# linusmossberg/monte-carlo-ray-tracer

Measured on AMD Instinct MI355X. Metric: Mray/s (whole node), 1920x1080 @ 256 spp path trace, higher is better.
Workload: dtype f64; 1 GPU; hexagon_room.json cam0 1920x1080 @ 256 spp (BASELINE configs[1]); width=1920, height=1080, spp=256, integrator=path_tracer, seed=305419896, frame_finite=True

## Files before the change

monte-carlo-ray-tracer_amd/csrc/mcrt_hip.hip:

```cpp
#include <hip/hip_runtime.h>

#include <algorithm>
#include <chrono>
#include <cstdio>
#include <cstring>
#include <map>
#include <memory>
#include <mutex>
#include <string>
#include <vector>

#include "../../include/mcrt.h"
#include "mcrt_integrator.hpp"
#include "mcrt_lanesm.hpp"
#include "mcrt_qbvh.hpp"
#include "mcrt_wavefront.hpp"
#include "mcrt_waveknn.hpp"
#include "mcrt_groupknn.hpp"
#include "mcrt_widerec.hpp"
#include "mcrt_layout.hpp"
#include "mcrt_internal.hpp"
#include "mcrt_aov.hpp"
#include "mcrt_plan.hpp"
#include "mcrt_select.hpp"
// ... 583 lines not shown
    DeviceOrder& o = g_device_order[(unsigned)ctx->device & 63u];
    std::lock_guard<std::mutex> guard(o.m);
    if (gpu_wait && o.owner && o.owner != ctx) {
        HIP_TRY(ctx, hipSetDevice(ctx->device));
        HIP_TRY(ctx, hipStreamWaitEvent(stream, o.last, 0));
    }
    const int rc = launchRenderImpl(ctx, cam, global_seed, integrator, d_out, stream, film_out, opt);
    if (rc == MCRT_OK && ctx->pending) {
        o.last = ctx->ev1;
        o.owner = ctx;
        if (cam != &ctx->last_cam) ctx->last_cam = *cam;
        ctx->last_seed = global_seed;
        ctx->last_integrator = integrator;
        ctx->last_out = d_out;
        ctx->last_film = film_out;
        ctx->last_stream = stream;
    }
    return rc;
}

int launchRenderImpl(mcrt_ctx* ctx, const mcrt_camera_desc* cam, uint32_t global_seed, int integrator, double* d_out, hipStream_t stream,
                     double* film_out, const RenderOptions& opt) {
    if (!ctx->has_scene) return fail(ctx, MCRT_ERR_NO_SCENE, "mcrt_render before mcrt_upload_scene");
    if (int rc = validateCamera(ctx, cam)) return rc;
    const bool photon = integrator == MCRT_INTEGRATOR_PHOTON_MAPPER;
    if (integrator != MCRT_INTEGRATOR_PATH_TRACER && !photon) return fail(ctx, MCRT_ERR_INVALID, "unknown integrator");
    if (photon && !ctx->has_photons) return fail(ctx, MCRT_ERR_NO_PHOTONS, "photon mapping render before mcrt_upload_photons");
    if (ctx->pending) return fail(ctx, MCRT_ERR_INVALID, "a render is already in flight: call mcrt_render_finish");
    HIP_TRY(ctx, hipSetDevice(ctx->device));
    ctx->lean_used = false;

    const uint32_t owned_rows = mcrt_shard_rows(cam, nullptr);
    FrameFacts frame;
    frame.photon = photon;
    frame.paths = (uint64_t)owned_rows * cam->width * cam->sqrtspp * cam->sqrtspp;
    frame.filtered = filmSplats(cam->film_filter, cam->film_radius);
    frame.film_out = film_out != nullptr;
    frame.k_nearest = ctx->k_nearest;
    frame.max_lds = (uint32_t)ctx->max_lds;
    frame.force_wf = ctx->force_wf;
    frame.force_pm_lane = ctx->force_pm_lane;
    const KernelChoice choice = selectKernel(ctx->facts, frame, opt);
    if (choice.err != MCRT_OK) return fail(ctx, choice.err, choice.message);
    if (choice.form == MCRT_KERNEL_WAVEFRONT || choice.form == MCRT_KERNEL_WAVEFRONT_PM)
        return launchWavefront(ctx, cam, global_seed, d_out, stream, opt, choice, film_out);

    const void* kernel = instanceAddress(choice.instance, choice.lean);
    if (!kernel) return fail(ctx, MCRT_ERR_INVALID, "internal error: no such lean kernel instance");
    const bool pm_wave = choice.form == MCRT_KERNEL_PM_WAVE;
    const bool flat_karg = choice.instance == kInstFlatK512 || choice.instance == kInstFlatK768;
    DeviceScene launch_scene = ctx->scene;
    const uint32_t lds_bytes = planMegaLds(launch_scene, choice, (uint32_t)ctx->max_lds);
    if (lds_bytes > ctx->max_lds) return fail(ctx, MCRT_ERR_INVALID, "LDS plan exceeds the device limit");
    LaunchGeom g;
    if (int rc = occupancyGrid(ctx, kernel, choice.block, lds_bytes, g)) return rc;
    if (int rc = ensureScratch(ctx, g.total_lanes, photon && !pm_wave)) return rc;
    if (int rc = ensureSpill(ctx, megaSpillEntries(ctx->scene, choice, g.total_lanes) * sizeof(StackEntry))) return rc;
    if (int rc = beginFrame(ctx, stream, owned_rows == 0 ? (uint32_t)MCRT_KERNEL_NONE : choice.form)) return rc;
    if (owned_rows == 0) return endFrame(ctx, stream);
    ctx->lean_used = choice.lean;

    PassPlan pp;
    if (int rc = planSampleStore(ctx, opt.sample_store_gb, cam->width, owned_rows, cam->sqrtspp * cam->sqrtspp, pp)) return rc;
    RenderParams prm;
    fillRenderParams(prm, *cam, global_seed, owned_rows, ctx->work_counter.as<unsigned long long>(), ctx->stats.as<unsigned long long>(),
                     ctx->spill.as<StackEntry>(), ctx->samples.as<double>(), g.total_lanes);
    if (photon) {
        setRenderMaps(prm, ctx->maps[0], ctx->maps[1], ctx->k_nearest, ctx->direct_visualization);
        prm.knn_res_d2 = ctx->knn_res_d2.as<double>();
        prm.knn_res_idx = ctx->knn_res_idx.as<uint32_t>();
        prm.knn_visit_d2 = ctx->knn_visit_d2.as<double>();
        prm.knn_visit_oct = ctx->knn_visit_oct.as<uint32_t>();
        prm.knn_max_visit = ctx->knn_visit_alloc;
    }
    PmExtra pmx;
    if (pm_wave) {
        HIP_TRY(ctx, ctx->pm_stage.reserve(pmStageBytes(g.total_lanes)));
        HIP_TRY(ctx, ctx->knn_spill.reserve(pmKnnSpillBytes(g.total_lanes)));
        if (pmIorsInMemory(choice)) HIP_TRY(ctx, ctx->pm_iors.reserve(pmIorsBytes(g.total_lanes)));
        fillPmExtra(pmx, waveMapView(ctx, 0), waveMapView(ctx, 1), choice, ctx->pm_stage.as<double>(), ctx->knn_spill.as<uint32_t>(), ctx->pm_iors.as<double>());
    }
    FlatPreArg pre;
    if (flat_karg) {
        memset(&pre, 0, sizeof(pre));
        memcpy(pre.v, ctx->flat_pre_host.data(), ctx->flat_pre_host.size() * sizeof(float));
    }
    for (uint32_t row = 0; row < owned_rows; row += pp.pass_rows) {
        setRenderPass(prm, row, pp.pass_rows, photon, opt.chunks);
        const uint32_t grid = (uint32_t)std::min<uint64_t>(g.grid, (prm.work_items + g.block - 1) / g.block);
        HIP_TRY(ctx, hipMemsetAsync(ctx->work_counter.p, 0, sizeof(unsigned long long), stream));
        if (pm_wave)
            hipLaunchKernelGGL(kernelAs<PmKernelT>(kernel), dim3(grid), dim3(g.block), g.lds_bytes, stream, launch_scene, prm, pmx);
        else if (flat_karg)
            hipLaunchKernelGGL(kernelAs<FlatKernelT>(kernel), dim3(grid), dim3(g.block), g.lds_bytes, stream, launch_scene, prm, pre);
        else
            hipLaunchKernelGGL(kernelAs<RenderKernelT>(kernel), dim3(grid), dim3(g.block), g.lds_bytes, stream, launch_scene, prm);
        ctx->launches++;
        if (int rc = launchPassEpilogue(ctx, stream, prm.samples, prm.pass_pixels, prm.spp, d_out, prm.row_base, cam->width)) return rc;
    }
    return endFrame(ctx, stream);
}


int planSampleStore(mcrt_ctx* ctx, double store_gb, uint32_t width, uint32_t owned_rows, uint32_t spp, PassPlan& pp) {
    double gb = store_gb;
    size_t free_b = 0, total_b = 0;
    if (hipMemGetInfo(&free_b, &total_b) == hipSuccess) gb = std::min(gb, 0.4 * (double)(free_b + ctx->samples.bytes) / 1e9);
    else (void)hipGetLastError();
    for (;;) {
        pp = planPasses(width, owned_rows, spp, gb);
        if (ctx->samples.bytes >= pp.store_bytes) return MCRT_OK;
        if (ctx->samples.alloc(pp.store_bytes) == hipSuccess) return MCRT_OK;
        (void)hipGetLastError();
        if (pp.pass_rows <= 8) return fail(ctx, MCRT_ERR_HIP, "out of device memory for the per-sample store of one 8-row pass");
        gb = std::min(gb, (double)pp.store_bytes / 1e9) * 0.5;
    }
}

int uploadMap(mcrt_ctx* ctx, int which, const mcrt_photon_map_desc* m) {
    PhotonMapView& v = ctx->maps[which];
    memset(&v, 0, sizeof(v));
    ctx->map_children_ptr[which] = nullptr;
    if (!m || m->num_octants == 0 || m->num_photons == 0) return MCRT_OK;
    if (m->num_photons > 0xFFFFFFFEull) return fail(ctx, MCRT_ERR_UNSUPPORTED, "photon map larger than 2^32-2 photons per GPU");
    if (!m->octant_bounds || !m->octant_start_data || !m->octant_contained_data || !m->octant_next_sibling || !m->octant_leaf || !m->photons)
        return fail(ctx, MCRT_ERR_INVALID, "photon map descriptor has null arrays");
    const size_t n = m->num_octants;
    std::vector<uint32_t> start(n), contained(n);
    for (size_t i = 0; i < n; i++) {
        if (m->octant_start_data[i] + m->octant_contained_data[i] > m->num_photons)
            return fail(ctx, MCRT_ERR_INVALID, "photon map octant range exceeds the photon array");
        start[i] = (uint32_t)m->octant_start_data[i];
        contained[i] = (uint32_t)m->octant_contained_data[i];
    }
    if (int rc = uploadArray(ctx, ctx->map_bounds[which], m->octant_bounds, n * 6)) return rc;
    if (int rc = uploadArray(ctx, ctx->map_start[which], start.data(), n)) return rc;
    if (int rc = uploadArray(ctx, ctx->map_contained[which], contained.data(), n)) return rc;
    if (int rc = uploadArray(ctx, ctx->map_next[which], m->octant_next_sibling, n)) return rc;
    if (int rc = uploadArray(ctx, ctx->map_leaf[which], m->octant_leaf, n)) return rc;
    if (int rc = uploadArray(ctx, ctx->map_photons[which], m->photons, (size_t)m->num_photons * 8)) return rc;
    {
        std::vector<WideRec> wide;
        uint32_t root_a = 0, root_m = 0;
        const int wrc = buildWideRecords(m, contained.data(), std::max<uint32_t>(ctx->k_nearest, 1u), wide, root_a, root_m);
        if (wrc == 1) return fail(ctx, MCRT_ERR_INVALID, "photon octant with more than 8 children");
        if (wrc == 2) return fail(ctx, MCRT_ERR_UNSUPPORTED, "photon map too large for 32-bit record indices");
        if (int rc = uploadArray(ctx, ctx->map_children[which], wide.data(), wide.size())) return rc;
        ctx->map_children_ptr[which] = ctx->map_children[which].as<WideRec>();
        ctx->map_root_a[which] = root_a;
        ctx->map_root_m[which] = root_m;
    }
    v.num_octants = m->num_octants;
    v.num_photons = m->num_photons;
    v.octant_bounds = ctx->map_bounds[which].as<double>();
    v.octant_start = ctx->map_start[which].as<uint32_t>();
    v.octant_contained = ctx->map_contained[which].as<uint32_t>();
    v.octant_next = ctx->map_next[which].as<uint32_t>();
    v.octant_leaf = ctx->map_leaf[which].as<uint8_t>();
    v.photons = ctx->map_photons[which].as<float>();
    return buildMapPositions(ctx, which, m->num_photons);
}

#include "mcrt_photon_device.hpp"

}

// ... 894 lines not shown
```

monte-carlo-ray-tracer_amd/csrc/mcrt_launch.hpp:

```cpp
#ifndef MCRT_LAUNCH_FRAME_SECTION
#define MCRT_LAUNCH_FRAME_SECTION

#include <algorithm>
#include <cstring>
#include <vector>

#include "../../include/mcrt.h"
#include "mcrt_plan.hpp"
#include "mcrt_wavefront.hpp"

namespace mcrt {

inline std::vector<double> filmCacheTable(const mcrt_camera_desc& cam) {
    std::vector<double> table(cam.film_cache_size);
    for (uint32_t i = 0; i < cam.film_cache_size; i++)
        table[i] = filmFilterFunction(filmViewType(cam.film_filter), (2.0 * (int)i) / (double)(cam.film_cache_size - 1));
    return table;
}
inline FilmView makeFilmView(const mcrt_camera_desc& cam, const double* cache, double* blob) {
    FilmView f;
    f.type = filmViewType(cam.film_filter);
    f.width = cam.width;
    f.height = cam.height;
    f.radius = cam.film_radius > 0.0 ? cam.film_radius : filmDefaultRadius(cam.film_filter);
    f.two_inv_radius = 2.0 / f.radius;
    f.cache_size = cam.film_cache_size;
    f.cache = f.cache_size ? cache : nullptr;
    f.inv_dx = f.cache_size ? (double)(f.cache_size - 1) / f.radius : 0.0;
    f.blob = blob;
    return f;
}

inline void fillWfFrame(WfFrame& fr, const mcrt_camera_desc& cam, uint32_t global_seed, const ChunkPlan& cp, double* samples, const FilmView* film,
                        double* iors_deep, uint32_t iors_depth) {
    memset(&fr, 0, sizeof(fr));
    fr.cam = cam;
    fr.global_seed = global_seed;
    fr.spp = cam.sqrtspp * cam.sqrtspp;
    fr.tiles_x = (cam.width + 7) / 8;
    fr.chunk_shift = cp.shift;
    fr.chunk = cp.chunk;
    fr.samples = samples;
    fr.film.type = MCRT_FILM_BOX;
    if (film) fr.film = *film;
    fr.iors_deep = iors_deep;
    fr.iors_deep_rows = iors_depth - (uint32_t)kMaxIors;
}
inline void setWfPass(WfFrame& fr, uint32_t row_base, uint32_t row_end) {
    fr.row_base = row_base;
    fr.row_end = row_end;
    fr.pass_pixels = (unsigned long long)(row_end - row_base) * fr.cam.width;
    fr.work_items = ((unsigned long long)fr.tiles_x * ((row_end - row_base + 7) / 8) * 64ull) << fr.chunk_shift;
}

inline std::vector<double> lightFlux(const mcrt_scene_desc& s) {
    std::vector<double> flux((size_t)s.num_lights * 3);
    for (uint32_t i = 0; i < s.num_lights; i++) {
        const uint32_t ls = s.light_surface[i];
        for (int c = 0; c < 3; c++) flux[(size_t)i * 3 + c] = s.materials[s.surf_material[ls]].emittance[c] * s.surf_area[ls];
    }
    return flux;
}
inline void planEmission(const std::vector<double>& flux, double emissions, double caustic_factor, std::vector<unsigned long long>& first,
                         std::vector<double>& photon_flux) {
    const size_t nl = flux.size() / 3, photon_emissions = (size_t)((double)(size_t)emissions * caustic_factor);
    double total_add_flux = 0.0;
    for (size_t i = 0; i < nl; i++) total_add_flux += 0.0 + flux[i * 3] + flux[i * 3 + 1] + flux[i * 3 + 2];
    first.assign(nl + 1, 0ull);
    photon_flux.resize(nl * 3);
    for (size_t i = 0; i < nl; i++) {
        const double* f = &flux[i * 3];
        const double share = (0.0 + f[0] + f[1] + f[2]) / total_add_flux;
        const size_t n = (size_t)((double)photon_emissions * share);
        first[i + 1] = first[i] + n;
        for (int c = 0; c < 3; c++) photon_flux[i * 3 + c] = f[c] / (double)n;
    }
}

}
#endif

#if defined(MCRT_LAUNCH_KERNEL_ARGS) && !defined(MCRT_LAUNCH_KERNEL_SECTION)
#define MCRT_LAUNCH_KERNEL_SECTION

inline void planStaging(DeviceScene& d, uint32_t max_lds, uint32_t flat_max, const HostLayout& L) {
    d.stage_all = 1;
    d.stage_nodes = 0;
    const uint32_t fixed = planLds(DeviceScene{}, kBlock).total;
    if (planLds(d, kBlock).total - fixed > 48u * 1024u || planLds(d, kBlock).total > max_lds || L.num_quadric_surfaces) {
        d.stage_all = 0;
        d.stage_nodes = std::min<uint32_t>(d.num_nodes, 512u);
    }
    d.flat = (d.stage_all && d.num_surfaces <= flat_max && !L.flat_prim.empty() && L.num_quadric_surfaces == 0) ? 1u : 0u;
}

constexpr uint32_t kPmStageNodes = 128;

inline SceneFacts sceneFacts(const DeviceScene& d, const HostLayout& L, const mcrt_scene_desc& s) {
    SceneFacts facts;
    facts.material_flags = 0u;
    for (uint32_t i = 0; i < s.num_materials; i++) facts.material_flags |= s.materials[i].flags;
    facts.q_single = L.q_single;
    facts.flat = d.flat != 0;
    facts.cull = d.flat_pre != nullptr;
    facts.cull_floats = L.flat_pre.size() == (size_t)d.pre_tri_pairs * kTriPairFloats + (size_t)d.pre_sph_pairs * kSphPairFloats ? (uint32_t)L.flat_pre.size() : 0u;
    facts.stage_all = d.stage_all != 0;
    facts.num_nodes = d.num_nodes;
    facts.q_nodes = d.q_nodes;
    DeviceScene pm = d;
    if (!pm.stage_all) pm.stage_nodes = std::min<uint32_t>(pm.stage_nodes, kPmStageNodes);
    for (uint32_t i = 0; i < 8; i++) {
        facts.pm_lds[0][i] = alignUp(planLds(pm, kBlock, true, 2 * (i + 1), kPmLdsIors).total, 16);
        facts.pm_lds[1][i] = alignUp(planLds(pm, 1024u, true, 2 * (i + 1), kPmLdsIors).total, 16);
    }
    facts.pm_lds_full = alignUp(planLds(pm, kBlock, true, kLdsStackDepth, kMaxIors).total, 16);
    return facts;
}

inline bool pmWide(const KernelChoice& c) { return c.instance >= kInstPMWide && c.instance <= kInstPMWide_CountAll; }
inline bool pmIorsInMemory(const KernelChoice& c) { return c.form == MCRT_KERNEL_PM_WAVE && (c.block == 1024u || pmWide(c)); }

inline uint32_t planMegaLds(DeviceScene& launch_scene, const KernelChoice& c, uint32_t max_lds) {
    if (c.form == MCRT_KERNEL_PM_WAVE) {
        if (!launch_scene.stage_all) launch_scene.stage_nodes = std::min<uint32_t>(launch_scene.stage_nodes, kPmStageNodes);
        const uint32_t knn_bytes = waveKnnBytes(pmWide(c) ? kWaveRowsLarge : kWaveRows) + (launch_scene.stage_all ? 0u : kWaveStateBytes);
        return alignUp(planLds(launch_scene, c.block, true, c.stack_depth, pmIorsInMemory(c) ? kPmLdsIors : (uint32_t)kMaxIors).total, 16) + (c.block / 64) * knn_bytes;
    }
    if (c.form == MCRT_KERNEL_LANE_SM) {
        const uint32_t fixed = planSmLds(DeviceScene{}, c.block, c.stack_depth).total;
        if (!launch_scene.stage_all && fixed < max_lds) launch_scene.stage_nodes = std::min<uint32_t>(launch_scene.stage_nodes, (max_lds - fixed) / 64u);
        return planSmLds(launch_scene, c.block, c.stack_depth).total;
    }
    return planLds(launch_scene, c.block, c.form != MCRT_KERNEL_FLAT).total;
}
inline size_t megaSpillEntries(const DeviceScene& d, const KernelChoice& c, uint32_t total_lanes) {
    const uint32_t in_lds = c.form == MCRT_KERNEL_PM_WAVE ? std::min<uint32_t>(c.stack_depth, kLdsStackDepth) : (uint32_t)kLdsStackDepth;
    return (size_t)total_lanes * (d.stack_depth - in_lds);
}

constexpr int kSmShadeLanes = 40, kSmRegenLanes = 16, kSmMinTrav = 20, kSmLeafLanes = 32, kSmMinInner = 8;

inline void fillRenderParams(RenderParams& prm, const mcrt_camera_desc& cam, uint32_t global_seed, uint32_t owned_rows, unsigned long long* work_counter,
                             unsigned long long* stats, StackEntry* spill, double* samples, uint32_t total_lanes) {
    memset(&prm, 0, sizeof(prm));
    prm.cam = cam;
    prm.global_seed = global_seed;
    prm.spp = cam.sqrtspp * cam.sqrtspp;
    prm.owned_rows = owned_rows;
    prm.tiles_x = (cam.width + 7) / 8;
    prm.tiles_y = (owned_rows + 7) / 8;
    prm.work_items = (uint64_t)prm.tiles_x * prm.tiles_y * 64ull;
    prm.work_counter = work_counter;
    prm.stats = stats;
    prm.spill = spill;
    prm.samples = samples;
    prm.total_lanes = total_lanes;
    prm.sm_shade_lanes = kSmShadeLanes;
    prm.sm_regen_lanes = kSmRegenLanes;
    prm.sm_min_trav = kSmMinTrav;
    prm.sm_leaf_lanes = kSmLeafLanes;
    prm.sm_min_inner = kSmMinInner;
    prm.sm_lds_depth = kLdsStackDepth;
}
inline void setRenderMaps(RenderParams& prm, const PhotonMapView& global_map, const PhotonMapView& caustic_map, uint32_t k_nearest, int direct_visualization) {
    prm.global_map = global_map;
    prm.caustic_map = caustic_map;
    prm.k_nearest = k_nearest;
    prm.direct_visualization = direct_visualization ? 1u : 0u;
}
inline void setRenderPass(RenderParams& prm, uint32_t row, uint64_t pass_rows, bool photon, long long chunks = -1) {
    prm.row_base = row;
    prm.row_end = (uint32_t)std::min<uint64_t>(prm.owned_rows, row + pass_rows);
    prm.pass_pixels = (uint64_t)(prm.row_end - prm.row_base) * prm.cam.width;
    const ChunkPlan cp = photon ? planChunks(prm.spp, unitsWanted(prm.total_lanes, 128, prm.pass_pixels, chunks))
                                : planChunksMega(prm.spp, prm.total_lanes, prm.pass_pixels, chunks);
    prm.chunk_shift = cp.shift;
    prm.chunk = cp.chunk;
    const uint64_t tiles = (uint64_t)prm.tiles_x * ((prm.row_end - prm.row_base + 7) / 8);
    prm.work_items = (tiles * 64ull) << cp.shift;
}

inline size_t pmStageBytes(uint32_t total_lanes) { return (size_t)kStageDoubles * total_lanes * sizeof(double); }
inline size_t pmKnnSpillBytes(uint32_t total_lanes) { return (size_t)(total_lanes / 64) * kWaveSpill * 3 * sizeof(uint32_t); }
inline size_t pmIorsBytes(uint32_t total_lanes) { return (size_t)kMaxIors * total_lanes * sizeof(double); }
inline void fillPmExtra(PmExtra& pmx, const PhotonMapViewW& global_map, const PhotonMapViewW& caustic_map, const KernelChoice& c, double* stage,
                        uint32_t* knn_spill, double* iors_global) {
    pmx.global_map = global_map;
    pmx.caustic_map = caustic_map;
// ... 152 lines not shown
```

monte-carlo-ray-tracer_amd/csrc/mcrt_layout.hpp:

```cpp
#pragma once

#include <algorithm>
#include <cmath>
#include <cstdlib>
#include <cstring>
#include <string>
#include <vector>

#include "../../include/mcrt.h"
#include "mcrt_scene.hpp"
#include "mcrt_qbvh.hpp"
#include "mcrt_bvh_shared.hpp"

namespace mcrt {

constexpr size_t kFlatCopyMax = 4096;

struct HostLayout {
    std::vector<double> node_bounds;
    std::vector<NodeMeta> node_meta;
    std::vector<double> prim;
    std::vector<double> normal;
    std::vector<double> shade_rec;
    bool any_vn = false;
// ... 145 lines not shown
    std::vector<uint32_t> order;
    order.reserve(n);
    std::vector<uint32_t> first_child_new(n, 0), child_count(n, 0);
    order.push_back(0);
    for (size_t head = 0; head < order.size(); head++) {
        const uint32_t old = order[head];
        if (s->node_num_surfaces[old] != 0) continue;
        uint32_t c = old + 1, cnt = 0;
        first_child_new[head] = (uint32_t)order.size();
        while (c != 0 && c < n) {
            order.push_back(c);
            cnt++;
            if (order.size() > n) {
                err = "BVH node links are cyclic";
                return MCRT_ERR_INVALID;
            }
            c = s->node_next_sibling[c];
        }
        child_count[head] = cnt;
    }
    if (order.size() != n) {
        err = "BVH has unreachable nodes";
        return MCRT_ERR_INVALID;
    }
    for (uint32_t i = 0; i < n; i++) {
        const uint32_t old = order[i];
        memcpy(&bounds[(size_t)i * 6], s->node_bounds + (size_t)old * 6, 48);
        if (s->node_num_surfaces[old] != 0) {
            if ((uint64_t)s->node_start_surface[old] + s->node_num_surfaces[old] > s->num_surfaces) {
                err = "BVH leaf range exceeds the surface array";
                return MCRT_ERR_INVALID;
            }
            meta[i] = NodeMeta{s->node_start_surface[old], s->node_num_surfaces[old]};
        } else {
            meta[i] = NodeMeta{first_child_new[i], kInnerFlag | child_count[i]};
        }
    }
    return MCRT_OK;
}

inline void buildFlatCull(HostLayout& L, uint32_t ns) {
    L.flat_pre.clear();
    L.pre_tri_pairs = L.pre_sph_pairs = 0;
    const uint32_t nt = L.flat_tris, nsph = ns - nt;
    if (ns == 0) return;
    double lo[3] = {INFINITY, INFINITY, INFINITY}, hi[3] = {-INFINITY, -INFINITY, -INFINITY};
    auto grow = [&](const double* p, double r) {
        for (int a = 0; a < 3; a++) {
            lo[a] = std::min(lo[a], p[a] - r);
            hi[a] = std::max(hi[a], p[a] + r);
        }
    };
    for (uint32_t i = 0; i < ns; i++) {
        const double* r = &L.flat_prim[(size_t)i * kPrimStride];
        if (i < nt) {
            const double v1[3] = {r[0] + r[3], r[1] + r[4], r[2] + r[5]}, v2[3] = {r[0] + r[6], r[1] + r[7], r[2] + r[8]};
            grow(r, 0.0);
            grow(v1, 0.0);
            grow(v2, 0.0);
        } else {
            grow(r, fabs(r[3]));
        }
    }
    double H = 0.0;
    for (int a = 0; a < 3; a++) {
        if (!(fabs(lo[a]) <= 1e7) || !(fabs(hi[a]) <= 1e7)) return;
        L.pre_centre[a] = 0.5 * (lo[a] + hi[a]);
        H = std::max(H, 0.5 * (hi[a] - lo[a]));
    }
    if (!(H > 0.0)) return;
    L.pre_bound = 4.0 * H;
    const double u = ldexp(1.0, -24), bound = L.pre_bound;
    auto up = [](double x) {
        float f = (float)x;
        if ((double)f < x) f = nextafterf(f, INFINITY);
        return f;
    };
    auto down = [](double x) {
        float f = (float)x;
        if ((double)f > x) f = nextafterf(f, -INFINITY);
        return f;
    };
    auto len = [](const double* v) { return sqrt(v[0] * v[0] + v[1] * v[1] + v[2] * v[2]); };
    L.pre_tri_pairs = (nt + 1) / 2;
    L.pre_sph_pairs = (nsph + 1) / 2;
    L.flat_pre.assign((size_t)L.pre_tri_pairs * kTriPairFloats + (size_t)L.pre_sph_pairs * kSphPairFloats, 0.0f);
    for (uint32_t i = 0; i < 2 * L.pre_tri_pairs; i++) {
        float* q = &L.flat_pre[(size_t)(i / 2) * kTriPairFloats + (i & 1)];
        if (i >= nt) {
            q[2 * 9] = -INFINITY;
            continue;
        }
        const double* r = &L.flat_prim[(size_t)i * kPrimStride];
        double a[3];
        for (int c = 0; c < 3; c++) a[c] = r[c] - L.pre_centre[c];
        for (int c = 0; c < 3; c++) q[2 * c] = (float)a[c];
        for (int c = 0; c < 6; c++) q[2 * (3 + c)] = (float)r[3 + c];
        const double e1 = len(r + 3), e2 = len(r + 6), tmax = sqrt(3.0) * bound + len(a);
        const double k = 4.0 * u;
        double eu = k * 31.0 * e1 * e2 * e2 * tmax, ev = k * 31.0 * e1 * e1 * e2 * tmax, et = k * 31.0 * e1 * e1 * e2 * e2 * tmax;
        double ew = k * 40.0 * e1 * e2 * ((e1 + e2) * tmax + e1 * e2);
        const bool degenerate = !(e1 > 1e-12) || !(e2 > 1e-12) || !(eu > 1e-30) || !(ev > 1e-30) || !(et > 1e-30) || !(ew > 1e-30);
        if (degenerate) eu = ev = et = ew = INFINITY;
        q[2 * 9] = up(eu);
        q[2 * 10] = up(ev);
        q[2 * 11] = up(et);
        q[2 * 12] = up(ew);
    }
    float* sph = L.flat_pre.data() + (size_t)L.pre_tri_pairs * kTriPairFloats;
    for (uint32_t i = 0; i < 2 * L.pre_sph_pairs; i++) {
        float* q = &sph[(size_t)(i / 2) * kSphPairFloats + (i & 1)];
        if (i >= nsph) {
            q[2 * 3] = -INFINITY;
            q[2 * 4] = 0.0f;
            continue;
        }
        const double* r = &L.flat_prim[(size_t)(nt + i) * kPrimStride];
        double c[3], cinf = 0.0;
        for (int a = 0; a < 3; a++) {
            c[a] = r[a] - L.pre_centre[a];
            cinf = std::max(cinf, fabs(c[a]));
            q[2 * a] = (float)c[a];
        }
        const double rad = fabs(r[3]), M = bound + cinf;
        const double beta = 4.0 * (12.0 * u + 7.0 * u * M / rad), gamma = 4.0 * (2.0 * u * rad * rad + 7.0 * u * rad * M);
        if (!(rad > 0.0) || !(beta < 0.25) || !(gamma > 1e-30)) {
            q[2 * 3] = INFINITY;
            q[2 * 4] = 0.0f;
        } else {
            q[2 * 3] = up(rad * rad + gamma);
            q[2 * 4] = down(1.0 - beta);
        }
    }
}


inline void synthRangeTree(const mcrt_scene_desc* s, std::vector<double>& bounds, std::vector<uint32_t>& start, std::vector<uint32_t>& count,
                           std::vector<uint32_t>& next) {
    const uint32_t ns = s->num_surfaces;
    std::vector<double> sb((size_t)ns * 6);
    for (uint32_t i = 0; i < ns; i++) surfaceBounds(s->surf_kind[i], s->surf_v + (size_t)i * 9, s->quadrics, &sb[(size_t)i * 6]);
    struct Rec {
        static uint32_t build(uint32_t a, uint32_t b, const std::vector<double>& sb, std::vector<double>& bounds, std::vector<uint32_t>& start,
                              std::vector<uint32_t>& count, std::vector<uint32_t>& next) {
            const uint32_t me = (uint32_t)start.size();
            double bb[6] = {1.7976931348623157e308, 1.7976931348623157e308, 1.7976931348623157e308,
                            -1.7976931348623157e308, -1.7976931348623157e308, -1.7976931348623157e308};
            for (uint32_t i = a; i < b; i++)
                for (int c = 0; c < 3; c++) {
                    bb[c] = sb[(size_t)i * 6 + c] < bb[c] ? sb[(size_t)i * 6 + c] : bb[c];
                    bb[3 + c] = sb[(size_t)i * 6 + 3 + c] > bb[3 + c] ? sb[(size_t)i * 6 + 3 + c] : bb[3 + c];
                }
            bounds.insert(bounds.end(), bb, bb + 6);
            start.push_back(a);
            next.push_back(0u);
            if (b - a <= 4u) {
                count.push_back(b - a);
                return me;
            }
            count.push_back(0u);
            const uint32_t part = (b - a + 3u) / 4u;
            uint32_t prev = 0;
            for (uint32_t x = a; x < b; x += part) {
                const uint32_t child = build(x, x + part < b ? x + part : b, sb, bounds, start, count, next);
                if (prev) next[prev] = child;
                prev = child;
            }
            return me;
        }
    };
    bounds.clear();
    start.clear();
    count.clear();
    next.clear();
    if (ns) Rec::build(0u, ns, sb, bounds, start, count, next);
}

inline int buildLayout(const mcrt_scene_desc* s, HostLayout& L, std::string& err) {
    const size_t ns = s->num_surfaces;
    L.prim.assign(ns * kPrimStride, 0.0);
    L.normal.assign(ns * 3, 0.0);
    L.any_vn = false;
    L.num_quadric_surfaces = 0;
    L.surf_v_patched.clear();
    for (size_t i = 0; i < ns; i++) {
        if (s->surf_material[i] >= s->num_materials) {
            err = "surface material index out of range";
            return MCRT_ERR_INVALID;
        }
        double* r = &L.prim[i * kPrimStride];
// ... 125 lines not shown
```

monte-carlo-ray-tracer_amd/csrc/mcrt_scene.hpp:

```cpp
#pragma once

#include "mcrt_math.hpp"

namespace mcrt {

constexpr uint32_t kInnerFlag = 0x80000000u;
constexpr int kPrimStride = 10;
constexpr int kLdsStackDepth = 16;
constexpr int kMaxStackDepth = 128;

struct NodeMeta {
    uint32_t a, b;
};

struct Node64 {
    double b[6];
    uint32_t a, m;
    uint32_t pad0, pad1;
};
constexpr uint32_t kSmInner = 0x100u;

struct Ray {
    d3 start, direction, inv_direction;
    double medium_ior, refraction_scale;
// ... 195 lines not shown
    const double tag = rec[9];
    if constexpr (kQuadrics) {
        if (tag == 3.0) return quadricIntersect(quadricPtr(rec[0]), ray, out);
    }
    if (tag == 1.0) {
        d3 so = ray.start - ld3(rec);
        double b = 2.0 * dot(ray.direction, so);
        double c = dot(so, so) - sq(rec[3]);
        double d = b * b - 4.0 * 1.0 * c;
        if (d < 0.0) return false;
        double sd = sqrt(d);
        double t = -0.5 * (b + (b < 0.0 ? -sd : sd));
        double t_min = t / 1.0;
        double t_max = c / t;
        if (t_min > t_max) {
            double tmp = t_min;
            t_min = t_max;
            t_max = tmp;
        }
        if (!(t_max >= 0.0)) return false;
        out.t = t_min < 0.0 ? t_max : t_min;
        out.u = 0.0;
        out.v = 0.0;
        out.interpolate = false;
        return true;
    }
    d3 v0 = ld3(rec), E1 = ld3(rec + 3), E2 = ld3(rec + 6);
    d3 P_ = cross(ray.direction, E2);
    double determinant = dot(P_, E1);
    if (determinant < kEpsilon && determinant > -kEpsilon) return false;
    double inv_determinant = 1.0 / determinant;
    d3 T = ray.start - v0;
    double u = dot(P_, T) * inv_determinant;
    if (u > 1.0 || u < 0.0) return false;
    d3 Q = cross(T, E1);
    double v = dot(Q, ray.direction) * inv_determinant;
    if (v > 1.0 || v < 0.0 || u + v > 1.0) return false;
    double t = dot(Q, E2) * inv_determinant;
    if (t <= 0.0) return false;
    out.t = t;
    out.interpolate = tag >= 2.0;
    out.u = out.interpolate ? u : 0.0;
    out.v = out.interpolate ? v : 0.0;
    return true;
}

MCRT_HD bool closer(double t, uint32_t surface, const Hit& best) {
    return t < best.t || (t == best.t && surface < best.surface);
}

template <class P>
MCRT_HD bool triangleTestFlat(P rec, d3 start, d3 direction, double& t, double& u, double& v) {
    d3 v0 = ld3(rec), E1 = ld3(rec + 3), E2 = ld3(rec + 6);
    d3 P_ = cross(direction, E2);
    double determinant = dot(P_, E1);
    double inv_determinant = 1.0 / determinant;
    d3 T = start - v0;
    u = dot(P_, T) * inv_determinant;
    d3 Q = cross(T, E1);
    v = dot(Q, direction) * inv_determinant;
    t = dot(Q, E2) * inv_determinant;
    const bool parallel = determinant < kEpsilon && determinant > -kEpsilon;
    const bool u_out = u > 1.0 || u < 0.0;
    const bool v_out = v > 1.0 || v < 0.0 || u + v > 1.0;
    return !parallel & !u_out & !v_out & !(t <= 0.0);
}
template <class P>
MCRT_HD bool sphereTestFlat(P rec, d3 start, d3 direction, double& t_hit) {
    d3 so = start - ld3(rec);
    double b = 2.0 * dot(direction, so);
    double c = dot(so, so) - sq(rec[3]);
    double d = b * b - 4.0 * 1.0 * c;
    double sd = sqrt(d);
    double t = -0.5 * (b + (b < 0.0 ? -sd : sd));
    double t_min = t / 1.0;
    double t_max = c / t;
    const bool swap = t_min > t_max;
    double lo = swap ? t_max : t_min, hi = swap ? t_min : t_max;
    t_hit = lo < 0.0 ? hi : lo;
    return !(d < 0.0) & (hi >= 0.0);
}

typedef float f2 __attribute__((vector_size(8)));
constexpr int kTriPairFloats = 32, kSphPairFloats = 16;
constexpr float kCullB2 = 1.0f + 8.0f * 5.9604645e-8f * 1.0001f;

template <class P>
MCRT_HD f2 ldf2(P p) {
    return f2{p[0], p[1]};
}

struct CullRay {
    f2 sx, sy, sz, dx, dy, dz;
    bool in_domain;
};
MCRT_HD CullRay cullRayAt(double cx, double cy, double cz, double bound, d3 start, d3 direction) {
    CullRay r;
    const double x = start.x - cx, y = start.y - cy, z = start.z - cz;
    r.in_domain = fabs(x) <= bound && fabs(y) <= bound && fabs(z) <= bound &&
                  (direction.x * direction.x + direction.y * direction.y + direction.z * direction.z) <= 1.000001;
    const float fx = (float)x, fy = (float)y, fz = (float)z;
    const float gx = (float)direction.x, gy = (float)direction.y, gz = (float)direction.z;
    r.sx = f2{fx, fx}; r.sy = f2{fy, fy}; r.sz = f2{fz, fz};
    r.dx = f2{gx, gx}; r.dy = f2{gy, gy}; r.dz = f2{gz, gz};
    return r;
}
template <bool kAll>
MCRT_HD CullRay cullRay(const SceneViewT<kAll>& sv, d3 start, d3 direction) {
    return cullRayAt(sv.pre_cx, sv.pre_cy, sv.pre_cz, sv.pre_bound, start, direction);
}

template <class P>
MCRT_HD uint32_t cullTriangles(P pre, uint32_t pairs, uint32_t count, const CullRay& r) {
#if defined(__clang__)
#pragma clang fp contract(fast)
#endif
    uint32_t rej = 0;
    for (uint32_t p = pairs; p-- > 0;) {
        P q = pre + (size_t)p * kTriPairFloats;
        const f2 ax = ldf2(q + 0), ay = ldf2(q + 2), az = ldf2(q + 4);
        const f2 e1x = ldf2(q + 6), e1y = ldf2(q + 8), e1z = ldf2(q + 10);
        const f2 e2x = ldf2(q + 12), e2y = ldf2(q + 14), e2z = ldf2(q + 16);
        const f2 eu = ldf2(q + 18), ev = ldf2(q + 20), et = ldf2(q + 22), ew = ldf2(q + 24);
        const f2 Px = r.dy * e2z - e2y * r.dz, Py = r.dz * e2x - e2z * r.dx, Pz = r.dx * e2y - e2x * r.dy;
        const f2 det = Px * e1x + Py * e1y + Pz * e1z;
        const f2 Tx = r.sx - ax, Ty = r.sy - ay, Tz = r.sz - az;
        const f2 uN = Px * Tx + Py * Ty + Pz * Tz;
        const f2 Qx = Ty * e1z - e1y * Tz, Qy = Tz * e1x - e1z * Tx, Qz = Tx * e1y - e1x * Ty;
        const f2 vN = Qx * r.dx + Qy * r.dy + Qz * r.dz;
        const f2 tN = Qx * e2x + Qy * e2y + Qz * e2z;
        const f2 A = uN * det + eu, B = vN * det + ev, C = tN * det + et;
        const f2 W = (det * det + ew) - (uN + vN) * det;
        const uint32_t x1 = floatBits(A[1]) | floatBits(B[1]) | floatBits(C[1]) | floatBits(W[1]);
        const uint32_t x0 = floatBits(A[0]) | floatBits(B[0]) | floatBits(C[0]) | floatBits(W[0]);
        rej = (rej << 1) | (x1 >> 31);
        rej = (rej << 1) | (x0 >> 31);
    }
    const uint32_t all = count >= 32u ? 0xFFFFFFFFu : ((1u << count) - 1u);
    return ((r.in_domain && pairs != 0u) ? ~rej : 0xFFFFFFFFu) & all;
}

template <class P>
MCRT_HD uint32_t cullSpheres(P pre, uint32_t pairs, uint32_t count, const CullRay& r) {
#if defined(__clang__)
#pragma clang fp contract(fast)
#endif
    uint32_t rej = 0;
    for (uint32_t p = pairs; p-- > 0;) {
        P q = pre + (size_t)p * kSphPairFloats;
        const f2 cx = ldf2(q + 0), cy = ldf2(q + 2), cz = ldf2(q + 4), cg = ldf2(q + 6), cb = ldf2(q + 8);
        const f2 ox = cx - r.sx, oy = cy - r.sy, oz = cz - r.sz;
        const f2 nb = ox * r.dx + oy * r.dy + oz * r.dz;
        const f2 so2 = ox * ox + oy * oy + oz * oz;
        const f2 inner = cg - so2 * cb;
        const f2 D = (nb * f2{kCullB2, kCullB2}) * nb + inner;
        const uint32_t x1 = (floatBits(nb[1]) & floatBits(inner[1])) | floatBits(D[1]);
        const uint32_t x0 = (floatBits(nb[0]) & floatBits(inner[0])) | floatBits(D[0]);
        rej = (rej << 1) | (x1 >> 31);
        rej = (rej << 1) | (x0 >> 31);
    }
    const uint32_t all = count >= 32u ? 0xFFFFFFFFu : ((1u << count) - 1u);
    return ((r.in_domain && pairs != 0u) ? ~rej : 0xFFFFFFFFu) & all;
}

MCRT_HD uint32_t lowestBit(uint32_t m) { return (uint32_t)__builtin_ctz(m); }

MCRT_HD void hitInit(Hit& h, double t_limit) {
    h.t = t_limit;
    h.u = 0.0;
    h.v = 0.0;
    h.surface = kNoSurface;
    h.interpolate = false;
}

struct ShadowQuery {
    uint32_t light;
    double t_near;
    double t_far;
    double dist;
    MCRT_HD void setRange(double d) {
        dist = d;
        t_near = d * (1.0 - 1e-9);
        t_far = d * (1.0 + 1e-9);
    }
};

template <bool kAll, bool kCount, bool kShadow, bool kFlat = false, bool kPreK = false>
MCRT_HD Hit sceneIntersect(const SceneViewT<kAll>& sv, const Ray& ray, const LaneStack& stk, TraceCounters& cnt,
                           const ShadowQuery* sq = nullptr) {
    Hit best;
    best.t = kDblMax;
    best.u = 0.0;
    best.v = 0.0;
    best.surface = kNoSurface;
    best.interpolate = false;
    cnt.rays++;
    uint32_t sh_light = kNoSurface;
    double sh_near = 0.0;

    if (kFlat || sv.num_nodes == 0) {
        if (kFlat || (kAll && sv.flat_prim)) {
            const uint32_t nt = sv.flat_tris, ns = sv.num_surfaces;
            if (kFlat || sv.pre_tri_pairs + sv.pre_sph_pairs != 0u) {
                const CullRay cr = cullRay(sv, ray.start, ray.direction);
                for (uint32_t base = 0; base < nt; base += 32u) {
                    const uint32_t left = nt - base, pairs_left = sv.pre_tri_pairs - base / 2u;
                    uint32_t mt;
                    if constexpr (kPreK)
                        mt = cullTriangles(sv.flat_pre_k + (size_t)(base / 2u) * kTriPairFloats, sv.pre_tri_pairs ? (pairs_left < 16u ? pairs_left : 16u) : 0u,
                                           left < 32u ? left : 32u, cr);
                    else
                        mt = cullTriangles(sv.flat_pre + (size_t)(base / 2u) * kTriPairFloats, sv.pre_tri_pairs ? (pairs_left < 16u ? pairs_left : 16u) : 0u,
                                           left < 32u ? left : 32u, cr);
                    if (kCount) cnt.prim_tests += (uint32_t)__builtin_popcount(mt);
                    while (mt) {
                        const uint32_t i = base + lowestBit(mt);
                        mt &= mt - 1u;
                        double t, u, v;
                        cptr<double, kAll> rec = sv.flat_prim + (size_t)i * kPrimStride;
                        const bool ok = triangleTestFlat(rec, ray.start, ray.direction, t, u, v);
                        const uint32_t idx = sv.flat_index[i];
                        if (ok && closer(t, idx, best)) {
                            const bool interp = rec[9] >= 2.0;
                            best.t = t;
                            best.u = interp ? u : 0.0;
                            best.v = interp ? v : 0.0;
                            best.interpolate = interp;
                            best.surface = idx;
                        }
                    }
                }
                cptr<float, kAll> spre = sv.flat_pre + (size_t)sv.pre_tri_pairs * kTriPairFloats;
                const float* spre_k = kPreK ? sv.flat_pre_k + (size_t)sv.pre_tri_pairs * kTriPairFloats : nullptr;
                for (uint32_t base = 0; base < ns - nt; base += 32u) {
                    const uint32_t left = ns - nt - base, pairs_left = sv.pre_sph_pairs - base / 2u;
                    uint32_t ms;
                    if constexpr (kPreK)
                        ms = cullSpheres(spre_k + (size_t)(base / 2u) * kSphPairFloats, sv.pre_sph_pairs ? (pairs_left < 16u ? pairs_left : 16u) : 0u,
                                         left < 32u ? left : 32u, cr);
                    else
                        ms = cullSpheres(spre + (size_t)(base / 2u) * kSphPairFloats, sv.pre_sph_pairs ? (pairs_left < 16u ? pairs_left : 16u) : 0u,
                                         left < 32u ? left : 32u, cr);
                    if (kCount) cnt.prim_tests += (uint32_t)__builtin_popcount(ms);
                    while (ms) {
                        const uint32_t i = nt + base + lowestBit(ms);
                        ms &= ms - 1u;
                        double t;
                        const bool ok = sphereTestFlat(sv.flat_prim + (size_t)i * kPrimStride, ray.start, ray.direction, t);
                        const uint32_t idx = sv.flat_index[i];
                        if (ok && closer(t, idx, best)) {
                            best.t = t;
                            best.u = 0.0;
                            best.v = 0.0;
                            best.interpolate = false;
                            best.surface = idx;
                        }
                    }
                }
                return best;
            }
            if constexpr (kFlat) return best;
#pragma unroll 2
            for (uint32_t i = 0; i < nt; i++) {
                double t, u, v;
                if (kCount) cnt.prim_tests++;
                cptr<double, kAll> rec = sv.flat_prim + (size_t)i * kPrimStride;
                const bool ok = triangleTestFlat(rec, ray.start, ray.direction, t, u, v);
                const uint32_t idx = sv.flat_index[i];
                if (ok && closer(t, idx, best)) {
                    const bool interp = rec[9] >= 2.0;
                    best.t = t;
                    best.u = interp ? u : 0.0;
                    best.v = interp ? v : 0.0;
                    best.interpolate = interp;
                    best.surface = idx;
                }
            }
#pragma unroll 2
            for (uint32_t i = nt; i < ns; i++) {
                double t;
                if (kCount) cnt.prim_tests++;
                const bool ok = sphereTestFlat(sv.flat_prim + (size_t)i * kPrimStride, ray.start, ray.direction, t);
                const uint32_t idx = sv.flat_index[i];
                if (ok && closer(t, idx, best)) {
                    best.t = t;
                    best.u = 0.0;
                    best.v = 0.0;
                    best.interpolate = false;
                    best.surface = idx;
                }
            }
            return best;
        }
        for (uint32_t i = 0; i < sv.num_surfaces; i++) {
            Hit h;
            if (kCount) cnt.prim_tests++;
            if (primIntersect<QuadricsIn<kAll>::value>(sv.prim + (size_t)i * kPrimStride, ray, h) && closer(h.t, i, best)) {
                best = h;
                best.surface = i;
                if (kShadow && i != sh_light && h.t < sh_near) return best;
            }
        }
        return best;
    }

    if (kShadow) {
        sh_light = sq->light;
        Hit h;
        if (kCount) cnt.prim_tests++;
        if (!primIntersect<QuadricsIn<kAll>::value>(sv.prim + (size_t)sh_light * kPrimStride, ray, h)) return best;
        best = h;
        best.surface = sh_light;
        sh_near = h.t;
    }

    const bool fast = finite64(ray.inv_direction.x) && finite64(ray.inv_direction.y) && finite64(ray.inv_direction.z);

    double t;
    if (kCount) cnt.node_tests++;
    {
        Box rb = loadBox(sv, 0u);
        if (!(fast ? boxIntersect<true>(rb, ray, t) : boxIntersect<false>(rb, ray, t))) return best;
    }

    int sp = 0;
    uint32_t node = 0;
    bool have = true;
    while (have) {
        NodeMeta m = loadMeta(sv, node);
        while (m.b & kInnerFlag) {
            const uint32_t first = m.a, count = m.b & ~kInnerFlag;
            double near_t = 0.0;
            uint32_t near_node = kNoSurface;
            for (uint32_t c = first; c < first + count; c++) {
                Box cb = loadBox(sv, c);
                if (kCount) cnt.node_tests++;
                const bool hit = fast ? boxIntersect<true>(cb, ray, t) : boxIntersect<false>(cb, ray, t);
                if (hit && t <= best.t) {
                    uint32_t push_node = c;
                    double push_t = t;
// ... 62 lines not shown
```

Before: 11030 Mray/s.

## Precompute triangle normal and cross terms for float cull test using Plücker form

Reformulates the per-pair float triangle cull test so that the geometric normal, its offset, and the edge-by-centre cross products are precomputed on the host. The ray moment is computed once per ray, so each triangle needs only dot products instead of per-triangle cross products. Error bounds are retuned for the shorter arithmetic. It also flattens the argument-block (kPreK) path into a single cull call per primitive type, restricted to at most 32 of each, with a host guard. The trade-off is a larger per-pair record (40 floats instead of 32), which means more loads and a bigger argument block, plus an unroll pragma on the cull loop.

```diff
diff --git a/monte-carlo-ray-tracer_amd/csrc/mcrt_hip.hip b/monte-carlo-ray-tracer_amd/csrc/mcrt_hip.hip
--- a/monte-carlo-ray-tracer_amd/csrc/mcrt_hip.hip
+++ b/monte-carlo-ray-tracer_amd/csrc/mcrt_hip.hip
@@ -689,6 +689,9 @@
     }
     FlatPreArg pre;
     if (flat_karg) {
+        if (launch_scene.pre_tri_pairs > kPreKMaxPairs || launch_scene.pre_sph_pairs > kPreKMaxPairs || ctx->flat_pre_host.size() > kFlatPreArgFloats ||
+            ctx->flat_pre_host.size() != (size_t)launch_scene.pre_tri_pairs * kTriPairFloats + (size_t)launch_scene.pre_sph_pairs * kSphPairFloats)
+            return fail(ctx, MCRT_ERR_INVALID, "internal error: the argument-block flat kernel was selected for a scene of more than 32 triangles or 32 spheres");
         memset(&pre, 0, sizeof(pre));
         memcpy(pre.v, ctx->flat_pre_host.data(), ctx->flat_pre_host.size() * sizeof(float));
     }
diff --git a/monte-carlo-ray-tracer_amd/csrc/mcrt_launch.hpp b/monte-carlo-ray-tracer_amd/csrc/mcrt_launch.hpp
--- a/monte-carlo-ray-tracer_amd/csrc/mcrt_launch.hpp
+++ b/monte-carlo-ray-tracer_amd/csrc/mcrt_launch.hpp
@@ -103,7 +103,8 @@
     facts.q_single = L.q_single;
     facts.flat = d.flat != 0;
     facts.cull = d.flat_pre != nullptr;
-    facts.cull_floats = L.flat_pre.size() == (size_t)d.pre_tri_pairs * kTriPairFloats + (size_t)d.pre_sph_pairs * kSphPairFloats ? (uint32_t)L.flat_pre.size() : 0u;
+    const bool one_word = d.pre_tri_pairs <= kPreKMaxPairs && d.pre_sph_pairs <= kPreKMaxPairs;
+    facts.cull_floats = one_word && L.flat_pre.size() == (size_t)d.pre_tri_pairs * kTriPairFloats + (size_t)d.pre_sph_pairs * kSphPairFloats ? (uint32_t)L.flat_pre.size() : 0u;
     facts.stage_all = d.stage_all != 0;
     facts.num_nodes = d.num_nodes;
     facts.q_nodes = d.q_nodes;
diff --git a/monte-carlo-ray-tracer_amd/csrc/mcrt_layout.hpp b/monte-carlo-ray-tracer_amd/csrc/mcrt_layout.hpp
--- a/monte-carlo-ray-tracer_amd/csrc/mcrt_layout.hpp
+++ b/monte-carlo-ray-tracer_amd/csrc/mcrt_layout.hpp
@@ -251,30 +251,45 @@
         return f;
     };
     auto len = [](const double* v) { return sqrt(v[0] * v[0] + v[1] * v[1] + v[2] * v[2]); };
+    auto cross3 = [](const double* x, const double* y, double* o) {
+        o[0] = x[1] * y[2] - x[2] * y[1];
+        o[1] = x[2] * y[0] - x[0] * y[2];
+        o[2] = x[0] * y[1] - x[1] * y[0];
+    };
     L.pre_tri_pairs = (nt + 1) / 2;
     L.pre_sph_pairs = (nsph + 1) / 2;
     L.flat_pre.assign((size_t)L.pre_tri_pairs * kTriPairFloats + (size_t)L.pre_sph_pairs * kSphPairFloats, 0.0f);
     for (uint32_t i = 0; i < 2 * L.pre_tri_pairs; i++) {
         float* q = &L.flat_pre[(size_t)(i / 2) * kTriPairFloats + (i & 1)];
         if (i >= nt) {
-            q[2 * 9] = -INFINITY;
+            q[2 * 16] = -INFINITY;
             continue;
         }
         const double* r = &L.flat_prim[(size_t)i * kPrimStride];
-        double a[3];
+        const double *E1 = r + 3, *E2 = r + 6;
+        double a[3], nd[3], g[3], h[3];
         for (int c = 0; c < 3; c++) a[c] = r[c] - L.pre_centre[c];
-        for (int c = 0; c < 3; c++) q[2 * c] = (float)a[c];
-        for (int c = 0; c < 6; c++) q[2 * (3 + c)] = (float)r[3 + c];
-        const double e1 = len(r + 3), e2 = len(r + 6), tmax = sqrt(3.0) * bound + len(a);
+        cross3(E2, E1, nd);
+        cross3(E2, a, g);
+        cross3(a, E1, h);
+        for (int c = 0; c < 3; c++) {
+            q[2 * c] = (float)nd[c];
+            q[2 * (4 + c)] = (float)E2[c];
+            q[2 * (7 + c)] = (float)g[c];
+            q[2 * (10 + c)] = (float)E1[c];
+            q[2 * (13 + c)] = (float)h[c];
+        }
+        q[2 * 3] = (float)(a[0] * nd[0] + a[1] * nd[1] + a[2] * nd[2]);
+        const double e1 = len(E1), e2 = len(E2), tmax = sqrt(3.0) * bound + len(a);
         const double k = 4.0 * u;
-        double eu = k * 31.0 * e1 * e2 * e2 * tmax, ev = k * 31.0 * e1 * e1 * e2 * tmax, et = k * 31.0 * e1 * e1 * e2 * e2 * tmax;
-        double ew = k * 40.0 * e1 * e2 * ((e1 + e2) * tmax + e1 * e2);
+        double eu = k * 19.0 * e1 * e2 * e2 * tmax, ev = k * 19.0 * e1 * e1 * e2 * tmax, et = k * 12.0 * e1 * e1 * e2 * e2 * tmax;
+        double ew = k * 20.0 * e1 * e2 * ((e1 + e2) * tmax + e1 * e2);
         const bool degenerate = !(e1 > 1e-12) || !(e2 > 1e-12) || !(eu > 1e-30) || !(ev > 1e-30) || !(et > 1e-30) || !(ew > 1e-30);
         if (degenerate) eu = ev = et = ew = INFINITY;
-        q[2 * 9] = up(eu);
-        q[2 * 10] = up(ev);
-        q[2 * 11] = up(et);
-        q[2 * 12] = up(ew);
+        q[2 * 16] = up(eu);
+        q[2 * 17] = up(ev);
+        q[2 * 18] = up(et);
+        q[2 * 19] = up(ew);
     }
     float* sph = L.flat_pre.data() + (size_t)L.pre_tri_pairs * kTriPairFloats;
     for (uint32_t i = 0; i < 2 * L.pre_sph_pairs; i++) {
diff --git a/monte-carlo-ray-tracer_amd/csrc/mcrt_scene.hpp b/monte-carlo-ray-tracer_amd/csrc/mcrt_scene.hpp
--- a/monte-carlo-ray-tracer_amd/csrc/mcrt_scene.hpp
+++ b/monte-carlo-ray-tracer_amd/csrc/mcrt_scene.hpp
@@ -301,7 +301,8 @@
 }
 
 typedef float f2 __attribute__((vector_size(8)));
-constexpr int kTriPairFloats = 32, kSphPairFloats = 16;
+constexpr int kTriPairFloats = 40, kSphPairFloats = 16;
+constexpr uint32_t kPreKMaxPairs = 16;
 constexpr float kCullB2 = 1.0f + 8.0f * 5.9604645e-8f * 1.0001f;
 
 template <class P>
@@ -311,6 +312,7 @@
 
 struct CullRay {
     f2 sx, sy, sz, dx, dy, dz;
+    f2 mx, my, mz;
     bool in_domain;
 };
 MCRT_HD CullRay cullRayAt(double cx, double cy, double cz, double bound, d3 start, d3 direction) {
@@ -322,6 +324,8 @@
     const float gx = (float)direction.x, gy = (float)direction.y, gz = (float)direction.z;
     r.sx = f2{fx, fx}; r.sy = f2{fy, fy}; r.sz = f2{fz, fz};
     r.dx = f2{gx, gx}; r.dy = f2{gy, gy}; r.dz = f2{gz, gz};
+    const float mx = fy * gz - fz * gy, my = fz * gx - fx * gz, mz = fx * gy - fy * gx;
+    r.mx = f2{mx, mx}; r.my = f2{my, my}; r.mz = f2{mz, mz};
     return r;
 }
 template <bool kAll>
@@ -335,21 +339,19 @@
 #pragma clang fp contract(fast)
 #endif
     uint32_t rej = 0;
+#pragma unroll 2
     for (uint32_t p = pairs; p-- > 0;) {
         P q = pre + (size_t)p * kTriPairFloats;
-        const f2 ax = ldf2(q + 0), ay = ldf2(q + 2), az = ldf2(q + 4);
-        const f2 e1x = ldf2(q + 6), e1y = ldf2(q + 8), e1z = ldf2(q + 10);
-        const f2 e2x = ldf2(q + 12), e2y = ldf2(q + 14), e2z = ldf2(q + 16);
-        const f2 eu = ldf2(q + 18), ev = ldf2(q + 20), et = ldf2(q + 22), ew = ldf2(q + 24);
-        const f2 Px = r.dy * e2z - e2y * r.dz, Py = r.dz * e2x - e2z * r.dx, Pz = r.dx * e2y - e2x * r.dy;
-        const f2 det = Px * e1x + Py * e1y + Pz * e1z;
-        const f2 Tx = r.sx - ax, Ty = r.sy - ay, Tz = r.sz - az;
-        const f2 uN = Px * Tx + Py * Ty + Pz * Tz;
-        const f2 Qx = Ty * e1z - e1y * Tz, Qy = Tz * e1x - e1z * Tx, Qz = Tx * e1y - e1x * Ty;
-        const f2 vN = Qx * r.dx + Qy * r.dy + Qz * r.dz;
-        const f2 tN = Qx * e2x + Qy * e2y + Qz * e2z;
-        const f2 A = uN * det + eu, B = vN * det + ev, C = tN * det + et;
-        const f2 W = (det * det + ew) - (uN + vN) * det;
+        const f2 ndx = ldf2(q + 0), ndy = ldf2(q + 2), ndz = ldf2(q + 4), and_ = ldf2(q + 6);
+        const f2 det = r.dz * ndz + (r.dy * ndy + r.dx * ndx);
+        const f2 tP = (r.sz * ndz + (r.sy * ndy + r.sx * ndx)) - and_;
+        const f2 e2x = ldf2(q + 8), e2y = ldf2(q + 10), e2z = ldf2(q + 12), gx = ldf2(q + 14), gy = ldf2(q + 16), gz = ldf2(q + 18);
+        const f2 uN = ((((r.mx * e2x + r.my * e2y) + r.mz * e2z) - r.dx * gx) - r.dy * gy) - r.dz * gz;
+        const f2 e1x = ldf2(q + 20), e1y = ldf2(q + 22), e1z = ldf2(q + 24), hx = ldf2(q + 26), hy = ldf2(q + 28), hz = ldf2(q + 30);
+        const f2 vP = ((((r.mx * e1x + r.my * e1y) + r.mz * e1z) + r.dx * hx) + r.dy * hy) + r.dz * hz;
+        const f2 eu = ldf2(q + 32), ev = ldf2(q + 34), et = ldf2(q + 36), ew = ldf2(q + 38);
+        const f2 A = uN * det + eu, B = ev - vP * det, C = et - tP * det;
+        const f2 W = (det * det + ew) - (uN - vP) * det;
         const uint32_t x1 = floatBits(A[1]) | floatBits(B[1]) | floatBits(C[1]) | floatBits(W[1]);
         const uint32_t x0 = floatBits(A[0]) | floatBits(B[0]) | floatBits(C[0]) | floatBits(W[0]);
         rej = (rej << 1) | (x1 >> 31);
@@ -422,16 +424,7 @@
             const uint32_t nt = sv.flat_tris, ns = sv.num_surfaces;
             if (kFlat || sv.pre_tri_pairs + sv.pre_sph_pairs != 0u) {
                 const CullRay cr = cullRay(sv, ray.start, ray.direction);
-                for (uint32_t base = 0; base < nt; base += 32u) {
-                    const uint32_t left = nt - base, pairs_left = sv.pre_tri_pairs - base / 2u;
-                    uint32_t mt;
-                    if constexpr (kPreK)
-                        mt = cullTriangles(sv.flat_pre_k + (size_t)(base / 2u) * kTriPairFloats, sv.pre_tri_pairs ? (pairs_left < 16u ? pairs_left : 16u) : 0u,
-                                           left < 32u ? left : 32u, cr);
-                    else
-                        mt = cullTriangles(sv.flat_pre + (size_t)(base / 2u) * kTriPairFloats, sv.pre_tri_pairs ? (pairs_left < 16u ? pairs_left : 16u) : 0u,
-                                           left < 32u ? left : 32u, cr);
-                    if (kCount) cnt.prim_tests += (uint32_t)__builtin_popcount(mt);
+                auto testTriangles = [&](uint32_t base, uint32_t mt) {
                     while (mt) {
                         const uint32_t i = base + lowestBit(mt);
                         mt &= mt - 1u;
@@ -448,19 +441,8 @@
                             best.surface = idx;
                         }
                     }
-                }
-                cptr<float, kAll> spre = sv.flat_pre + (size_t)sv.pre_tri_pairs * kTriPairFloats;
-                const float* spre_k = kPreK ? sv.flat_pre_k + (size_t)sv.pre_tri_pairs * kTriPairFloats : nullptr;
-                for (uint32_t base = 0; base < ns - nt; base += 32u) {
-                    const uint32_t left = ns - nt - base, pairs_left = sv.pre_sph_pairs - base / 2u;
-                    uint32_t ms;
-                    if constexpr (kPreK)
-                        ms = cullSpheres(spre_k + (size_t)(base / 2u) * kSphPairFloats, sv.pre_sph_pairs ? (pairs_left < 16u ? pairs_left : 16u) : 0u,
-                                         left < 32u ? left : 32u, cr);
-                    else
-                        ms = cullSpheres(spre + (size_t)(base / 2u) * kSphPairFloats, sv.pre_sph_pairs ? (pairs_left < 16u ? pairs_left : 16u) : 0u,
-                                         left < 32u ? left : 32u, cr);
-                    if (kCount) cnt.prim_tests += (uint32_t)__builtin_popcount(ms);
+                };
+                auto testSpheres = [&](uint32_t base, uint32_t ms) {
                     while (ms) {
                         const uint32_t i = nt + base + lowestBit(ms);
                         ms &= ms - 1u;
@@ -475,6 +457,29 @@
                             best.surface = idx;
                         }
                     }
+                };
+                if constexpr (kPreK) {
+                    const uint32_t mt = cullTriangles(sv.flat_pre_k, sv.pre_tri_pairs, nt, cr);
+                    const uint32_t ms = cullSpheres(sv.flat_pre_k + (size_t)sv.pre_tri_pairs * kTriPairFloats, sv.pre_sph_pairs, ns - nt, cr);
+                    if (kCount) cnt.prim_tests += (uint32_t)__builtin_popcount(mt) + (uint32_t)__builtin_popcount(ms);
+                    testTriangles(0u, mt);
+                    testSpheres(0u, ms);
+                    return best;
+                }
+                for (uint32_t base = 0; base < nt; base += 32u) {
+                    const uint32_t left = nt - base, pairs_left = sv.pre_tri_pairs - base / 2u;
+                    const uint32_t mt = cullTriangles(sv.flat_pre + (size_t)(base / 2u) * kTriPairFloats, sv.pre_tri_pairs ? (pairs_left < 16u ? pairs_left : 16u) : 0u,
+                                                      left < 32u ? left : 32u, cr);
+                    if (kCount) cnt.prim_tests += (uint32_t)__builtin_popcount(mt);
+                    testTriangles(base, mt);
+                }
+                cptr<float, kAll> spre = sv.flat_pre + (size_t)sv.pre_tri_pairs * kTriPairFloats;
+                for (uint32_t base = 0; base < ns - nt; base += 32u) {
+                    const uint32_t left = ns - nt - base, pairs_left = sv.pre_sph_pairs - base / 2u;
+                    const uint32_t ms = cullSpheres(spre + (size_t)(base / 2u) * kSphPairFloats, sv.pre_sph_pairs ? (pairs_left < 16u ? pairs_left : 16u) : 0u,
+                                                    left < 32u ? left : 32u, cr);
+                    if (kCount) cnt.prim_tests += (uint32_t)__builtin_popcount(ms);
+                    testSpheres(base, ms);
                 }
                 return best;
             }
```

New measurement: 11500 Mray/s (median of 6 runs). 4.2% higher.
